# mzhaoshuai/CenterCLIP

Measured on AMD Instinct MI355X. Metric: clips/sec (ViT-B/32, 12f), higher is better.
Workload: dtype fp16 (MFMA operands; fp32 accumulate, residual stream, LN, softmax; cluster + similarity fp32); 1 GPU; cfg2 MSR-VTT-shaped: ViT-B/32 224^2, 12 frames -> 3 segments @block 7, K=49, batch 16, 32 words; global_batch=16, parallelism=single GPU

## Files before the change

### centerclip_amd/csrc/cluster.hip

```cpp
#include "cc_common.h"
#include "cc_kernels.h"

typedef float f32x4 __attribute__((ext_vector_type(4)));

__global__ __launch_bounds__(256) void token_norm_kernel(const float* __restrict__ x, cc_token_layout lay,
                                                         int P, int N, int W, float* __restrict__ sqn,
                                                         float* __restrict__ nrm, float* __restrict__ inv,
                                                         float* __restrict__ xn, int* __restrict__ chunkmax,
                                                         int nchunks) {
    (void)chunkmax; (void)nchunks;
    const int lane = threadIdx.x & 63;
    const int bpp = (N + 3) >> 2;
    const int p = ((int)blockIdx.x >> 3) / bpp * 8 + ((int)blockIdx.x & 7);
    const int j = (((int)blockIdx.x >> 3) % bpp) * 4 + (threadIdx.x >> 6);
    if (p >= P || j >= N) return;
    const int tok = p * N + j;
    const float* src = cc_token_ptr(x, lay, p, j);
    float acc = 0.f;
    for (int w = lane * 4; w < W; w += 256) {
        const float4 v = *reinterpret_cast<const float4*>(src + w);
        acc = fmaf(v.x, v.x, acc);
        acc = fmaf(v.y, v.y, acc);
        acc = fmaf(v.z, v.z, acc);
        acc = fmaf(v.w, v.w, acc);
// ... 448 lines not shown
    return max(max(a, b), max(c, d));
}

__device__ __forceinline__ unsigned cc_wave_umin(unsigned v) {
    v = min(v, (unsigned)__builtin_amdgcn_update_dpp(-1, (int)v, 0xB1, 0xF, 0xF, false));
    v = min(v, (unsigned)__builtin_amdgcn_update_dpp(-1, (int)v, 0x4E, 0xF, 0xF, false));
    v = min(v, (unsigned)__builtin_amdgcn_update_dpp(-1, (int)v, 0x141, 0xF, 0xF, false));
    v = min(v, (unsigned)__builtin_amdgcn_update_dpp(-1, (int)v, 0x140, 0xF, 0xF, false));
    const unsigned a = __builtin_amdgcn_readlane(v, 0), b = __builtin_amdgcn_readlane(v, 16);
    const unsigned c = __builtin_amdgcn_readlane(v, 32), d = __builtin_amdgcn_readlane(v, 48);
    return min(min(a, b), min(c, d));
}

struct GatherDesc {
    const float* x; int64_t in_tok, in_frame;
    int B, T, T_new, n, W, K, mode;
    const long long* medoids; int med_stride;
    const long long* assign;
    const float* cluster_embed;
    const float* cls_mult;
    float* out; int64_t out_tok, out_frame;
    _Float16* h16; float* stats; float* shift;
};
template <bool LEFT>
__device__ void reduce_row_wave(const GatherDesc& g, int row, int lane, const int* med_lds);

struct SelStep {
    const long long* init;
    const int* done;
    int accumulate_iters;
};

#define SEL_WAVES 16
#define SEL_THREADS (64 * SEL_WAVES)
template <bool IN_LDS, int NE>
__global__ __launch_bounds__(SEL_THREADS) void kmedoids_select_kernel(const float* __restrict__ dist_in, float* dist_rw,
                                                              const float* __restrict__ norms,
                                                              const int* __restrict__ chunkmax, int slots_pp, int chunk,
                                                              int apply_shift, int N, int K, int iter_limit,
                                                              int id_sort, long long* __restrict__ medoids_out,
                                                              long long* __restrict__ assign_out,
                                                              int* __restrict__ iters_out, GatherDesc gd, SelStep step) {
    extern __shared__ __attribute__((aligned(16))) unsigned char smem_raw[];
    if (step.done && step.done[(int)blockIdx.x / chunk]) {
        if (step.init != medoids_out)
            for (int k = threadIdx.x; k < K; k += SEL_THREADS) medoids_out[(int64_t)blockIdx.x * K + k] = step.init[(int64_t)blockIdx.x * K + k];
        return;
    }
    const int E = (N + 63) >> 6;
    SelSmem s;
    {
        unsigned char* q = smem_raw;
        s.D = reinterpret_cast<float*>(q);
        if (IN_LDS) q += cc_align_up((size_t)N * N * 4, 8);
        s.best = reinterpret_cast<unsigned long long*>(q); q += cc_align_up((size_t)K * 8, 128);
        s.med = reinterpret_cast<int*>(q); q += cc_align_up((size_t)K * 4, 8);
        s.asg = reinterpret_cast<unsigned short*>(q); q += cc_align_up((size_t)N * 2, 8);
        s.order = reinterpret_cast<unsigned short*>(q); q += cc_align_up((size_t)N * 2, 8);
        s.prev = reinterpret_cast<unsigned short*>(q); q += cc_align_up((size_t)N * 2, 8);
        s.list = reinterpret_cast<unsigned short*>(q); q += cc_align_up((size_t)N * 2, 8);
        s.dirty = reinterpret_cast<unsigned char*>(q); q += cc_align_up((size_t)K, 8);
        s.count = reinterpret_cast<int*>(q); q += 8;
        s.cmask = reinterpret_cast<unsigned long long*>(q); q += (size_t)K * E * 8;
        s.mem = reinterpret_cast<unsigned int*>(q); q += cc_align_up((size_t)N * 4, 8);
        s.cnt = reinterpret_cast<unsigned short*>(q); q += cc_align_up((size_t)K * 2, 8);
        s.off = reinterpret_cast<unsigned short*>(q);
    }
    const int p = blockIdx.x;
    const int tid = threadIdx.x, lane = tid & 63, wave = tid >> 6;
    const int64_t base = (int64_t)p * N * N;
    const float* Dg = dist_in + base;
    SEL_PROF_INIT();
    SEL_STAMP(0);

    float shift_mx = 0.f;
    if (apply_shift) {
        int* red = reinterpret_cast<int*>(smem_raw);
        const int c0 = (p / chunk) * chunk, c1 = min((int)gridDim.x, c0 + chunk);
        int m = (int)0x80000000;
        for (int64_t q = (int64_t)c0 * slots_pp + tid; q < (int64_t)c1 * slots_pp; q += SEL_THREADS) m = max(m, chunkmax[q]);
        m = cc_wave_imax(m);
        if (lane == 0) red[wave] = m;
        __syncthreads();
        int mm = red[0];
#pragma unroll
        for (int w = 1; w < SEL_WAVES; ++w) mm = max(mm, red[w]);
        shift_mx = cc_ordered_int_to_float(mm);
        __syncthreads();
    }
    if (IN_LDS) {
        const float mx = shift_mx;
        float* dst = IN_LDS ? s.D : (dist_rw + base);
        const int total = N * N;
        if (IN_LDS && (total & 3) == 0) {
            const float4* src4 = reinterpret_cast<const float4*>(Dg);
            float4* dst4 = reinterpret_cast<float4*>(dst);
            const int total4 = total >> 2;
            for (int i0 = tid; i0 < total4; i0 += SEL_THREADS * 8) {
                float4 v[8];
#pragma unroll
                for (int u = 0; u < 8; ++u) {
                    const int idx = i0 + u * SEL_THREADS;
                    v[u] = idx < total4 ? src4[idx] : make_float4(0.f, 0.f, 0.f, 0.f);
                }
#pragma unroll
                for (int u = 0; u < 8; ++u) {
                    const int idx = i0 + u * SEL_THREADS;
                    if (idx < total4) {
                        if (apply_shift) {
                            v[u].x = (v[u].x - mx) - 1.0f; v[u].y = (v[u].y - mx) - 1.0f;
                            v[u].z = (v[u].z - mx) - 1.0f; v[u].w = (v[u].w - mx) - 1.0f;
                        }
                        dst4[idx] = v[u];
                    }
                }
            }
        } else {
            for (int i0 = tid; i0 < total; i0 += SEL_THREADS * 8) {
                float v[8];
#pragma unroll
                for (int u = 0; u < 8; ++u) {
                    const int idx = i0 + u * SEL_THREADS;
                    v[u] = idx < total ? Dg[idx] : 0.f;
                }
#pragma unroll
                for (int u = 0; u < 8; ++u) {
                    const int idx = i0 + u * SEL_THREADS;
                    if (idx < total) dst[idx] = apply_shift ? (v[u] - mx) - 1.0f : v[u];
                }
            }
        }
        if (!IN_LDS) Dg = dist_rw + base;
        __threadfence_block();
        __syncthreads();
        if (apply_shift) {
            float* dd = IN_LDS ? s.D : (dist_rw + base);
            for (int i = tid; i < N; i += SEL_THREADS) dd[(int64_t)i * N + i] -= 1.0f;
            __threadfence_block();
        }
        __syncthreads();
    }
    auto dread_global = [&](int i, int j) {
        float d = Dg[(int64_t)i * N + j];
        if (apply_shift) {
            d = (d - shift_mx) - 1.0f;
            if (i == j) d -= 1.0f;
        }
        return d;
    };
#define DREAD(i, j) (IN_LDS ? s.D[(i) * N + (j)] : dread_global((i), (j)))
    SEL_STAMP(1);

    for (int j = tid; j < N; j += SEL_THREADS) s.order[sum_rank(j, N)] = (unsigned short)j;

    if (step.init) {
        for (int k = tid; k < K; k += SEL_THREADS) s.med[k] = (int)step.init[(int64_t)p * K + k];
    } else if (wave == 0) {
        constexpr int TPL = NE;
        float nearest[TPL];
        const float* nr = norms + (int64_t)p * N;
        const int n0 = lane * TPL;
        const float NEG = -__builtin_inff();
#pragma unroll
        for (int e = 0; e < TPL; ++e) nearest[e] = (n0 + e < N) ? nr[n0 + e] : NEG;
        for (int i = 0; i < K; ++i) {
            float loc = nearest[0];
            int slot = 0;
#pragma unroll
            for (int e = 1; e < TPL; ++e)
                if (nearest[e] > loc) { loc = nearest[e]; slot = e; }
            float mx = fmaxf(loc, cc_dpp_f32<0xB1>(loc));
            mx = fmaxf(mx, cc_dpp_f32<0x4E>(mx));
            mx = fmaxf(mx, cc_dpp_f32<0x141>(mx));
            mx = fmaxf(mx, cc_dpp_f32<0x140>(mx));
            {
                const int iv = __float_as_int(mx);
                const float r0 = __int_as_float(__builtin_amdgcn_readlane(iv, 0)), r1 = __int_as_float(__builtin_amdgcn_readlane(iv, 16));
                const float r2 = __int_as_float(__builtin_amdgcn_readlane(iv, 32)), r3 = __int_as_float(__builtin_amdgcn_readlane(iv, 48));
                mx = fmaxf(fmaxf(r0, r1), fmaxf(r2, r3));
            }
            const int src = __ffsll((long long)__ballot(loc == mx)) - 1;
            const int m = src * TPL + __builtin_amdgcn_readlane(slot, src);
            if (lane == 0) s.med[i] = m;
            bool done = false;
            if constexpr (IN_LDS && TPL == 4) {
                if ((N & 3) == 0) {
                    const float4 r = *reinterpret_cast<const float4*>(s.D + m * N + min(n0, N - 4));
                    if (n0 < N) {
                        nearest[0] = (i == 0) ? r.x : fminf(nearest[0], r.x);
                        nearest[1] = (i == 0) ? r.y : fminf(nearest[1], r.y);
                        nearest[2] = (i == 0) ? r.z : fminf(nearest[2], r.z);
                        nearest[3] = (i == 0) ? r.w : fminf(nearest[3], r.w);
                    }
                    done = true;
                }
            }
            if (!done) {
                constexpr int RB = TPL <= 16 ? TPL : 8;
#pragma unroll
                for (int e0 = 0; e0 < TPL; e0 += RB) {
                    float r[RB];
#pragma unroll
                    for (int e = 0; e < RB; ++e) r[e] = (e0 + e < TPL) ? DREAD(m, min(n0 + e0 + e, N - 1)) : 0.f;
#pragma unroll
                    for (int e = 0; e < RB; ++e)
                        if (e0 + e < TPL && n0 + e0 + e < N)
                            nearest[e0 + e] = (i == 0) ? r[e] : fminf(nearest[e0 + e], r[e]);
                }
            }
        }
    }
    __syncthreads();
    SEL_STAMP(2);

    auto assign_step = [&](bool build_masks) {
        if (!IN_LDS && build_masks)
            for (int q = tid; q < K * E; q += SEL_THREADS) s.cmask[q] = 0ull;
        const int part = tid & 3, kq = (K + 3) >> 2;
        const int kb = part * kq, ke = min(K, kb + kq);
        for (int nb = 0; nb < N; nb += SEL_THREADS / 4) {
            const int n = nb + (tid >> 2);
            const int nn = min(n, N - 1);
            float best = __builtin_inff();
            int a = K;
            int k = kb;
            for (; k + 8 <= ke; k += 8) {
                int mk[8];
                float v[8];
#pragma unroll
                for (int u = 0; u < 8; ++u) mk[u] = s.med[k + u];
#pragma unroll
                for (int u = 0; u < 8; ++u) v[u] = DREAD(mk[u], nn);
#pragma unroll
                for (int u = 0; u < 8; ++u)
                    if (v[u] < best || a == K) { best = v[u]; a = k + u; }
            }
            for (; k < ke; ++k) {
                const float v = DREAD(s.med[k], nn);
                if (v < best || a == K) { best = v; a = k; }
            }
#pragma unroll
            for (int o = 1; o <= 2; o <<= 1) {
                const float ob = __shfl_xor(best, o, 64);
                const int oa = __shfl_xor(a, o, 64);
                if (oa < K && (a == K || ob < best || (ob == best && oa < a))) { best = ob; a = oa; }
            }
            if (n < N && part == 0) s.asg[n] = (unsigned short)a;
        }
        if (!IN_LDS && build_masks) {
            __syncthreads();
            for (int t = tid; t < N; t += SEL_THREADS)
                atomicOr(&s.cmask[(size_t)s.asg[s.order[t]] * E + (t >> 6)], 1ull << (t & 63));
        }
    };

    int iters = 0;
    long long ph0 = 0, ph1 = 0, ph2 = 0;
    for (int it = 0; it < iter_limit; ++it) {
        long long tq0 = 0, tq1 = 0, tq2 = 0;
        if (prof) tq0 = (long long)__builtin_readcyclecounter();
        assign_step(true);
        __syncthreads();
        if (prof) tq1 = (long long)__builtin_readcyclecounter();
        for (int k = tid; k < K; k += SEL_THREADS) s.dirty[k] = (it == 0) ? 1 : 0;
        if (tid == 0) *s.count = 0;
        __syncthreads();
        for (int n = tid; n < N; n += SEL_THREADS) {
            const unsigned short a = s.asg[n], pa = s.prev[n];
            if (it > 0 && a != pa) { s.dirty[a] = 1; s.dirty[pa] = 1; }
            s.prev[n] = a;
        }
        __syncthreads();
        if constexpr (!IN_LDS) {
        for (int k = tid; k < K; k += SEL_THREADS) {
            const unsigned long long* cm = s.cmask + (size_t)k * E;
            int n = 0;
            for (int w = 0; w < E; ++w) n += __popcll(cm[w]);
            s.cnt[k] = (unsigned short)n;
            if (s.dirty[k]) s.best[k] = ~0ull;
        }
        __syncthreads();
        if (wave == 0) {
            int carry = 0;
            for (int base = 0; base < K; base += 64) {
                const int v = (base + lane < K) ? (int)s.cnt[base + lane] : 0;
                int incl = v;
#pragma unroll
                for (int o = 1; o < 64; o <<= 1) {
                    const int up = __shfl_up(incl, o, 64);
                    if (lane >= o) incl += up;
                }
                if (base + lane < K) s.off[base + lane] = (unsigned short)(carry + incl - v);
                carry += __shfl(incl, 63, 64);
            }
            if (lane == 0) s.off[K] = (unsigned short)carry;
        }
        __syncthreads();
        const int vec_end = (N < 8) ? 0 : (N & ~7);
        const int rest = (N >> 5) << 5;
        auto tree_code = [&](int j) {
            return ((j & 7) << 7) | (j >= rest ? 31 : ((((j >> 3) & 3) << 5) | (j >> 9)));
        };
        for (int t = tid; t < N; t += SEL_THREADS) {
            const int j = s.order[t];
            const int a = s.asg[j];
            const unsigned long long* cm = s.cmask + (size_t)a * E;
            const int wt = t >> 6;
            unsigned long long below = cm[wt] & ((1ull << (t & 63)) - 1ull);
            int pos = s.off[a] + __popcll(below);
            int tp = below ? 64 * wt + 63 - __clzll((long long)below) : -1;
            for (int w = wt - 1; w >= 0; --w) {
                const unsigned long long m = cm[w];
                pos += __popcll(m);
                if (tp < 0 && m) tp = 64 * w + 63 - __clzll((long long)m);
            }
            unsigned e = (unsigned)j;
            if (j < vec_end) {
                const int jp = tp >= 0 ? (int)s.order[tp] : -1;
                const int x = (jp < 0 || jp >= vec_end) ? 0x3FF : (tree_code(j) ^ tree_code(jp));
                e |= (x ? SEL_F1 : 0u) | ((x >> 5) ? SEL_F2 : 0u) | ((x >> 7) ? SEL_F3 : 0u) | SEL_TREE |
                     (j >= rest ? SEL_LEFT : 0u);
            }
            s.mem[pos] = e;
        }
        __syncthreads();
        if (prof) tq2 = (long long)__builtin_readcyclecounter();
        for (int i = tid; i < N; i += SEL_THREADS) {
            const int cl = s.asg[i];
            if (!s.dirty[cl]) continue;
            const int b0 = s.off[cl], b1 = s.off[cl + 1];
            float c = 0.f, P = 0.f, R = 0.f, F = 0.f;
            for (int q = b0; q < b1; q += 8) {
                int e[8];
                float v[8];
#pragma unroll
                for (int u = 0; u < 8; ++u) e[u] = (q + u < b1) ? (int)s.mem[q + u] : -1;
#pragma unroll
                for (int u = 0; u < 8; ++u) {
                    const float d = DREAD(i, (e[u] < 0 ? 0 : e[u]) & (int)SEL_TOK);
                    v[u] = e[u] < 0 ? 0.f : d;
                }
#pragma unroll
                for (int u = 0; u < 8; ++u) {
                    const int ev = e[u] < 0 ? 0 : e[u];
                    const int m1 = -((ev >> 13) & 1), m2 = -((ev >> 14) & 1), m3 = -((ev >> 15) & 1);
                    const int mt = -((ev >> 16) & 1), ml = -((ev >> 17) & 1);
                    const float t1 = sel_and(c, m1);  P += t1;  c -= t1;
                    const float t2 = sel_and(P, m2);  R += t2;  P -= t2;
                    const float t3 = sel_and(R, m3);  F += t3;  R -= t3;
                    const float vt = sel_and(v[u], mt);
                    const float vl = sel_and(vt, ml);
                    P += vl;
                    c += vt - vl;
                    F += v[u] - vt;
                }
            }
            P += c; R += P; F += R;
            atomicMin(&s.best[cl], ((unsigned long long)cc_float_to_ordered_uint(F) << 32) | (unsigned)i);
        }
        __syncthreads();
        } else {
        for (int k = tid; k < K; k += SEL_THREADS)
            if (s.dirty[k]) s.best[k] = ~0ull;
        for (int n = tid; n < N; n += SEL_THREADS)
            if (s.dirty[s.asg[n]]) s.list[atomicAdd(s.count, 1)] = (unsigned short)n;
        __syncthreads();
        if (prof) tq2 = (long long)__builtin_readcyclecounter();
        {
            const int lq = tid & 7, slot = tid >> 3;
            const int M = *s.count;
            if (N >= 8) {
                const int vec_end = N & ~7, vs = N >> 3, passes = vs >> 2, nleft = vs & 3, ntail = N - vec_end;
                for (int i0 = 0; i0 < M; i0 += SEL_THREADS / 8) {
                    if (i0 + wave * 8 >= M) continue;
                    const int idx = i0 + slot;
                    const int i = s.list[min(idx, M - 1)];
                    const int cl = s.asg[i];
                    float c0[4] = {0.f, 0.f, 0.f, 0.f}, c1[4] = {0.f, 0.f, 0.f, 0.f};
                    const int p0 = min(passes, 16);
#pragma unroll 2
                    for (int it2 = 0; it2 < p0; ++it2) {
                        float d[4];
                        int a4[4];
#pragma unroll
                        for (int k = 0; k < 4; ++k) {
                            const int j = 32 * it2 + 8 * k + lq;
                            d[k] = s.D[i * N + j];
                            a4[k] = s.asg[j];
                        }
#pragma unroll
                        for (int k = 0; k < 4; ++k) c0[k] += (a4[k] == cl) ? d[k] : 0.f;
                    }
#pragma unroll 2
                    for (int it2 = 16; it2 < passes; ++it2) {
                        float d[4];
                        int a4[4];
#pragma unroll
                        for (int k = 0; k < 4; ++k) {
                            const int j = 32 * it2 + 8 * k + lq;
                            d[k] = s.D[i * N + j];
                            a4[k] = s.asg[j];
                        }
#pragma unroll
                        for (int k = 0; k < 4; ++k) c1[k] += (a4[k] == cl) ? d[k] : 0.f;
                    }
                    float P[4];
#pragma unroll
                    for (int k = 0; k < 4; ++k) P[k] = (passes > 16) ? c0[k] + c1[k] : c0[k];
                    for (int v = 0; v < nleft; ++v) {
                        const int j = 32 * passes + 8 * v + lq;
                        const float d = s.D[i * N + j];
                        P[0] += ((int)s.asg[j] == cl) ? d : 0.f;
                    }
                    const float R = ((P[0] + P[1]) + P[2]) + P[3];
                    float F = 0.f;
                    float dt[7];
                    int at[7];
#pragma unroll
                    for (int t = 0; t < 7; ++t) {
                        const int j = min(vec_end + t, N - 1);
                        dt[t] = s.D[i * N + j];
                        at[t] = s.asg[j];
                    }
#pragma unroll
                    for (int t = 0; t < 7; ++t)
                        if (t < ntail) F += (at[t] == cl) ? dt[t] : 0.f;
                    const int base = (tid & 63) & ~7;
                    float r8[8];
#pragma unroll
                    for (int l = 0; l < 8; ++l) r8[l] = __shfl(R, base + l, 64);
#pragma unroll
                    for (int l = 0; l < 8; ++l) F += r8[l];
                    if (lq == 0 && idx < M)
                        atomicMin(&s.best[cl], ((unsigned long long)cc_float_to_ordered_uint(F) << 32) | (unsigned)i);
                }
            } else {
                for (int q = tid; q < M; q += SEL_THREADS) {
                    const int i = s.list[q];
                    const int cl = s.asg[i];
                    float F = 0.f;
                    for (int t = 0; t < N; ++t) {
                        const int j = s.order[t];
                        const float d = DREAD(i, j);
                        F += (s.asg[j] == cl) ? d : 0.f;
                    }
                    atomicMin(&s.best[cl], ((unsigned long long)cc_float_to_ordered_uint(F) << 32) | (unsigned)i);
                }
            }
        }
        __syncthreads();
        }
        int changed = 0;
        for (int k = tid; k < K; k += SEL_THREADS) {
            const unsigned long long b = s.best[k];
            const int bi = (b == ~0ull) ? 0 : (int)(unsigned)(b & 0xFFFFFFFFull);
            changed |= (bi != s.med[k]);
            s.med[k] = bi;
        }
        ++iters;
        const int any_changed = __syncthreads_or(changed);
        if (prof) { ph0 += tq1 - tq0; ph1 += tq2 - tq1; ph2 += (long long)__builtin_readcyclecounter() - tq2; }
        if (!any_changed) break;
    }
    SEL_STAMP(3);

    if (id_sort) {
        int mine = 0, rank = 0;
        if (tid < K) {
            mine = s.med[tid];
            for (int q = 0; q < K; ++q) {
                const int o = s.med[q];
                rank += (o < mine || (o == mine && q < tid)) ? 1 : 0;
            }
        }
        __syncthreads();
        if (tid < K) s.med[rank] = mine;
        __syncthreads();
        if (assign_out) assign_step(false);
        __syncthreads();
    }
    for (int k = tid; k < K; k += SEL_THREADS) medoids_out[(int64_t)p * K + k] = s.med[k];
    if (assign_out)
        for (int n = tid; n < N; n += SEL_THREADS) assign_out[(int64_t)p * N + n] = (iter_limit > 0 || id_sort) ? s.asg[n] : 0;
    if (iters_out && tid == 0) iters_out[p] = step.accumulate_iters ? iters_out[p] + iters : iters;
    if (gd.out) {
        const int b = p % gd.B, sgm = p / gd.B, Lout = 1 + K;
        const int row0 = (b * gd.T_new + sgm) * Lout;
        for (int l = wave; l < Lout; l += SEL_WAVES) reduce_row_wave<false>(gd, row0 + l, lane, s.med);
    }
    SEL_STAMP(4);
    if (prof && tid == 0) {
        prof[(int64_t)blockIdx.x * 16 + 5] = iters;
        prof[(int64_t)blockIdx.x * 16 + 6] = ph0;
        prof[(int64_t)blockIdx.x * 16 + 7] = ph1;
        prof[(int64_t)blockIdx.x * 16 + 8] = ph2;
    }
#undef DREAD
}

struct CascadeSum {
    float4 a0, a1, a2;
    int chunk;
    __device__ __forceinline__ void init() {
        a0 = a1 = a2 = make_float4(0.f, 0.f, 0.f, 0.f);
        chunk = -1;
    }
    static __device__ __forceinline__ void acc(float4& d, const float4& v) { d.x += v.x; d.y += v.y; d.z += v.z; d.w += v.w; }
    __device__ __forceinline__ void close_chunk(int next_chunk) {
        acc(a1, a0);
        a0 = make_float4(0.f, 0.f, 0.f, 0.f);
        if ((chunk >> 4) != (next_chunk >> 4)) { acc(a2, a1); a1 = make_float4(0.f, 0.f, 0.f, 0.f); }
    }
    __device__ __forceinline__ void add(int row, const float4& v) {
        const int c = row >> 4;
        if (chunk >= 0 && c != chunk) close_chunk(c);
        chunk = c;
        acc(a0, v);
    }
    __device__ __forceinline__ float4 total(int rows) {
        if (chunk >= 0 && chunk < (rows >> 4)) {
            const int next = ((chunk >> 4) < (rows >> 8)) ? chunk + 16 : chunk;
            close_chunk(next);
        }
        float4 r = a0;
        acc(r, a1);
        acc(r, a2);
        return r;
    }
};

template <bool LEFT>
struct OuterSum {
    CascadeSum s0;
    CascadeSum s1, s2, s3;
    float4 l0, l1, l2;
    bool ilp;
    int rows4;
    __device__ __forceinline__ void init(bool left_columns, int rows) {
        s0.init();
        ilp = LEFT && left_columns;
        rows4 = (rows >> 2) << 2;
        if (LEFT) {
            s1.init(); s2.init(); s3.init();
            l0 = l1 = l2 = make_float4(0.f, 0.f, 0.f, 0.f);
        }
    }
    __device__ __forceinline__ void add(int row, const float4& v) {
        if (!LEFT || !ilp) { s0.add(row, v); return; }
        if (row >= rows4) {
            const int t = row - rows4;
            if (t == 0) l0 = v; else if (t == 1) l1 = v; else l2 = v;
            return;
        }
        const int a = row & 3, r = row >> 2;
        if (a == 0) s0.add(r, v); else if (a == 1) s1.add(r, v); else if (a == 2) s2.add(r, v); else s3.add(r, v);
    }
    __device__ __forceinline__ float4 total(int rows) {
        if (!LEFT || !ilp) return s0.total(rows);
        const int size = rows >> 2;
        float4 r = s0.total(size);
        CascadeSum::acc(r, l0); CascadeSum::acc(r, l1); CascadeSum::acc(r, l2);
        float4 t = s1.total(size); CascadeSum::acc(r, t);
        t = s2.total(size); CascadeSum::acc(r, t);
        t = s3.total(size); CascadeSum::acc(r, t);
        return r;
    }
};

__global__ __launch_bounds__(256) void cross_dist_kernel(const float* __restrict__ x1, const float* __restrict__ x2, int N1,
                                                         int N2, int W, int metric, float p, float* __restrict__ dist,
                                                         unsigned* __restrict__ gmax) {
    __shared__ float a[16][65], b[16][65];
    const int tid = threadIdx.x, ti = tid >> 4, tj = tid & 15;
    const int bz = blockIdx.z, i0 = blockIdx.y * 16, j0 = blockIdx.x * 16;
    const float* X = x1 + (int64_t)bz * N1 * W;
    const float* Y = x2 + (int64_t)bz * N2 * W;
    const bool gram = metric == CC_METRIC_COSINE || p == 2.0f;
    float dot = 0.f, nx = 0.f, ny = 0.f, lp = 0.f;
    for (int k0 = 0; k0 < W; k0 += 64) {
        for (int e = tid; e < 16 * 64; e += 256) {
            const int r = e >> 6, c = e & 63;
            a[r][c] = (i0 + r < N1 && k0 + c < W) ? X[(int64_t)(i0 + r) * W + k0 + c] : 0.f;
            b[r][c] = (j0 + r < N2 && k0 + c < W) ? Y[(int64_t)(j0 + r) * W + k0 + c] : 0.f;
        }
        __syncthreads();
        const int kn = min(64, W - k0);
        if (gram) {
            for (int c = 0; c < kn; ++c) {
                const float u = a[ti][c], v = b[tj][c];
                dot += u * v; nx += u * u; ny += v * v;
            }
        } else if (p == 1.0f) {
            for (int c = 0; c < kn; ++c) lp += fabsf(a[ti][c] - b[tj][c]);
        } else {
            for (int c = 0; c < kn; ++c) lp += powf(fabsf(a[ti][c] - b[tj][c]), p);
        }
        __syncthreads();
    }
    float d;
    if (metric == CC_METRIC_COSINE) d = 1.0f - dot / ((sqrtf(nx) + 1e-6f) * (sqrtf(ny) + 1e-6f));
    else if (p == 2.0f) d = sqrtf(fmaxf((nx + ny) - 2.f * dot, 0.f));
    else d = (p == 1.0f) ? lp : powf(lp, 1.0f / p);
    const bool in = i0 + ti < N1 && j0 + tj < N2;
    if (in) dist[((int64_t)bz * N1 + i0 + ti) * N2 + j0 + tj] = d;
    if (gmax) {
        float m = in ? d : -__builtin_inff();
        m = cc_wave_max(m);
        if ((tid & 63) == 0) atomicMax(gmax, cc_float_to_ordered_uint(m));
    }
}

__global__ __launch_bounds__(256) void cross_shift_kernel(float* __restrict__ dist, int P, int N1, int N2,
                                                          const unsigned* __restrict__ gmax, int self_nearest) {
    float mx = 0.f;
    if (gmax) {
        const unsigned u = *gmax;
        mx = __uint_as_float((u & 0x80000000u) ? (u & 0x7fffffffu) : ~u);
    }
    const int64_t total = (int64_t)P * N1 * N2;
    for (int64_t idx = (int64_t)blockIdx.x * 256 + threadIdx.x; idx < total; idx += (int64_t)gridDim.x * 256) {
        const int j = (int)(idx % N2);
        const int i = (int)((idx / N2) % N1);
        float v = dist[idx];
        if (gmax) v = (v - mx) - 1.0f;
        if (self_nearest && i == j) v -= 1.0f;
        dist[idx] = v;
    }
}

template <bool LEFT>
__device__ void reduce_row_wave(const GatherDesc& gd, int row, int lane, const int* med_lds) {
    const float* __restrict__ x = gd.x;
    const int64_t in_tok = gd.in_tok, in_frame = gd.in_frame, out_tok = gd.out_tok, out_frame = gd.out_frame;
    const int B = gd.B, T = gd.T, T_new = gd.T_new, n = gd.n, W = gd.W, K = gd.K, mode = gd.mode;
    const long long* __restrict__ medoids = gd.medoids;
    const int med_stride = gd.med_stride;
    const long long* __restrict__ assign = gd.assign;
    const float* __restrict__ cluster_embed = gd.cluster_embed;
    const float* __restrict__ cls_mult = gd.cls_mult;
    float* __restrict__ out = gd.out;
    _Float16* __restrict__ h16 = gd.h16;
    float* __restrict__ stats = gd.stats;
    float* __restrict__ shift = gd.shift;
    const int Lout = (mode == 2) ? 1 + n : 1 + K;
    float st_t = 0.f;
    float* own_row = nullptr;
    auto emit = [&](int w, const float4& v) {
        (void)w;
// ... 88 lines not shown
            a.x = a.x / den; a.y = a.y / den; a.z = a.z / den; a.w = a.w / den;
            if (emb) {
                const float4 e = *reinterpret_cast<const float4*>(emb + w);
                a.x += e.x; a.y += e.y; a.z += e.z; a.w += e.w;
            }
            *reinterpret_cast<float4*>(dst + w) = a;
            emit(w, a);
        }
    }
    finish();
}

template <bool LEFT>
__global__ __launch_bounds__(256) void reduce_tokens_kernel(GatherDesc gd) {
    const int row = blockIdx.x * 4 + (threadIdx.x >> 6);
    const int Lout = (gd.mode == 2) ? 1 + gd.n : 1 + gd.K;
    if (row >= gd.B * gd.T_new * Lout) return;
    reduce_row_wave<LEFT>(gd, row, threadIdx.x & 63, nullptr);
}

static GatherDesc gather_desc(const float* x, int64_t in_tok, int64_t in_frame, int B, int T, int T_new, int n, int W, int K,
                              int mode, const long long* medoids, int med_stride, const long long* assign,
                              const float* cluster_embed, const float* cls_mult, float* out, int64_t out_tok,
                              int64_t out_frame, _Float16* h16, float* stats, float* shift) {
    GatherDesc g{};
    g.x = x; g.in_tok = in_tok; g.in_frame = in_frame;
    g.B = B; g.T = T; g.T_new = T_new; g.n = n; g.W = W; g.K = K; g.mode = mode;
    g.medoids = medoids; g.med_stride = med_stride; g.assign = assign;
    g.cluster_embed = cluster_embed; g.cls_mult = cls_mult;
    g.out = out; g.out_tok = out_tok; g.out_frame = out_frame;
    g.h16 = h16; g.stats = stats; g.shift = shift;
    return g;
}

static void launch_reduce_tokens(hipStream_t st, const float* x, int64_t in_tok, int64_t in_frame, int B, int T, int T_new,
                                 int n, int W, int K, int mode, const long long* medoids, int med_stride,
                                 const long long* assign, const float* cluster_embed, const float* cls_mult, float* out,
                                 int64_t out_tok, int64_t out_frame, _Float16* h16, float* stats, float* shift) {
    const GatherDesc g = gather_desc(x, in_tok, in_frame, B, T, T_new, n, W, K, mode, medoids, med_stride, assign,
                                     cluster_embed, cls_mult, out, out_tok, out_frame, h16, stats, shift);
    const int rows = B * T_new * ((mode == 2) ? 1 + n : 1 + K);
    if (W & 31) hipLaunchKernelGGL(reduce_tokens_kernel<true>, dim3((rows + 3) / 4), dim3(256), 0, st, g);
    else hipLaunchKernelGGL(reduce_tokens_kernel<false>, dim3((rows + 3) / 4), dim3(256), 0, st, g);
}

namespace {

struct ClusterWs {
    int* tilemax;
    int slots_pp;
    int* chunkmax;
    float* sqn;
    float* nrm;
    float* inv;
    float* draw;
    float* xn;
    long long* med;
    long long* asg;
    long long* med2;
    int* done;
    size_t total;
};

struct SpectralWs {
    float* lap;
    float* q;
    int k4;
    void* eig;
    size_t eig_bytes;
    void* km;
    size_t km_bytes;
    size_t total;
};
ClusterWs carve(void* ws, int P, int N, int W, int pre_norm, int K_for_med);
extern "C" size_t cc_spectral_embedding_workspace_bytes(int32_t P, int32_t N);
SpectralWs carve_spectral(void* ws, int P, int N, int K) {
    SpectralWs s{};
    size_t off = 0;
    auto take = [&](size_t bytes) {
        void* ptr = ws ? static_cast<char*>(ws) + off : nullptr;
        off += cc_align_up(bytes, 256);
        return ptr;
    };
    s.k4 = (K + 3) / 4 * 4;
    s.lap = static_cast<float*>(take((size_t)P * N * N * sizeof(float)));
    s.q = static_cast<float*>(take((size_t)P * N * s.k4 * sizeof(float)));
    s.eig_bytes = cc_spectral_embedding_workspace_bytes(P, N);
    s.eig = take(s.eig_bytes);
    s.km_bytes = carve(nullptr, P, N, s.k4, 1, N).total;
    s.km = take(s.km_bytes);
    s.total = off;
    return s;
}

ClusterWs carve(void* ws, int P, int N, int W, int pre_norm, int K_for_med) {
    ClusterWs c{};
    size_t off = 0;
    auto take = [&](size_t bytes) {
        void* ptr = ws ? static_cast<char*>(ws) + off : nullptr;
        off += cc_align_up(bytes, 256);
        return ptr;
    };
    {
        const size_t nt = (size_t)(N + GT - 1) / GT;
        c.slots_pp = (int)(nt * (nt + 1) / 2 * 4);
        c.tilemax = static_cast<int*>(take((size_t)P * c.slots_pp * 4));
        c.chunkmax = static_cast<int*>(take((size_t)P * 4));
    }
    c.sqn = static_cast<float*>(take((size_t)P * N * 4));
    c.nrm = static_cast<float*>(take((size_t)P * N * 4));
    c.inv = static_cast<float*>(take((size_t)P * N * 4));
    c.draw = static_cast<float*>(take((size_t)P * N * N * 4));
    c.med = static_cast<long long*>(take((size_t)P * (size_t)K_for_med * 8));
    c.asg = static_cast<long long*>(take((size_t)P * N * 8));
    c.med2 = static_cast<long long*>(take((size_t)P * (size_t)K_for_med * 8));
    c.done = static_cast<int*>(take((size_t)P * 4));
    c.xn = pre_norm ? static_cast<float*>(take((size_t)P * N * W * 4)) : nullptr;
    c.total = off;
    return c;
}

bool layout_ok(const cc_token_layout* l, int W) {
    if (!l || l->B <= 0 || l->S <= 0 || l->fd <= 0 || l->n <= 0) return false;
    if (W <= 0 || (W & 3)) return false;
    return !((l->stride_b | l->stride_s | l->stride_f | l->stride_i) & 3);
}

cc_token_layout contiguous_layout(int P, int N, int W) {
    cc_token_layout l;
    l.B = P; l.S = 1; l.fd = 1; l.n = N;
    l.stride_b = (int64_t)N * W; l.stride_s = 0; l.stride_f = 0; l.stride_i = W;
    return l;
}

int run_distance(const float* x, cc_token_layout lay, int W, int metric, float p, int chunk, int pre_norm,
                 const ClusterWs& c, hipStream_t st) {
    const int P = lay.B * lay.S, N = lay.fd * lay.n;
    const int nb = ((P + 7) / 8) * 8 * ((N + 3) / 4);
    if (pre_norm) {
        hipLaunchKernelGGL(token_norm_kernel, dim3(nb), dim3(256), 0, st, x, lay, P, N, W, c.sqn, c.nrm, c.inv, c.xn,
                           (int*)nullptr, 0);
        x = c.xn;
        lay = contiguous_layout(P, N, W);
    }
    const bool own_norms = (metric == CC_METRIC_COSINE || p == 2.0f);
    if (!own_norms) {
        hipLaunchKernelGGL(token_norm_kernel, dim3(nb), dim3(256), 0, st, x, lay, P, N, W, c.sqn, c.nrm, c.inv,
                           (float*)nullptr, (int*)nullptr, 0);
        CC_LAUNCH_CHECK();
    }
    const int nt = (N + GT - 1) / GT;
    dim3 grid((unsigned)(((P + 7) / 8) * 8 * (nt * (nt + 1) / 2)));
    const size_t gram_smem = (size_t)2 * 2 * 2 * GT * GK * sizeof(_Float16) + 2 * GT * sizeof(float);
    if (metric == CC_METRIC_COSINE || p == 2.0f) {
        static bool configured = false;
        if (!configured) {
            if (hipFuncSetAttribute(reinterpret_cast<const void*>(gram_dist_kernel<CC_METRIC_COSINE>),
                                    hipFuncAttributeMaxDynamicSharedMemorySize, (int)gram_smem) != hipSuccess ||
                hipFuncSetAttribute(reinterpret_cast<const void*>(gram_dist_kernel<CC_METRIC_EUCLIDEAN>),
                                    hipFuncAttributeMaxDynamicSharedMemorySize, (int)gram_smem) != hipSuccess)
                return CC_ERR_HIP;
            configured = true;
        }
    }
    if (metric == CC_METRIC_COSINE) {
        hipLaunchKernelGGL(gram_dist_kernel<CC_METRIC_COSINE>, grid, dim3(256), gram_smem, st, x, lay, N, W, c.sqn, c.nrm,
                           c.inv, own_norms ? 1 : 0, c.draw, c.tilemax, chunk, nt, P);
    } else if (p == 2.0f) {
        hipLaunchKernelGGL(gram_dist_kernel<CC_METRIC_EUCLIDEAN>, grid, dim3(256), gram_smem, st, x, lay, N, W, c.sqn,
                           c.nrm, c.inv, own_norms ? 1 : 0, c.draw, c.tilemax, chunk, nt, P);
    } else if (p == 1.0f) {
        hipLaunchKernelGGL(lp_dist_kernel<1>, grid, dim3(256), 0, st, x, lay, N, W, p, c.draw, c.tilemax, chunk, nt, P);
    } else if (p > 3.0e38f) {
        hipLaunchKernelGGL(lp_dist_kernel<2>, grid, dim3(256), 0, st, x, lay, N, W, p, c.draw, c.tilemax, chunk, nt, P);
    } else {
        hipLaunchKernelGGL(lp_dist_kernel<0>, grid, dim3(256), 0, st, x, lay, N, W, p, c.draw, c.tilemax, chunk, nt, P);
    }
    CC_LAUNCH_CHECK();
    return CC_OK;
}

int run_distance_sq(const float* x, cc_token_layout lay, int W, const ClusterWs& c, hipStream_t st) {
    const int P = lay.B * lay.S, N = lay.fd * lay.n;
    const int nt = (N + GT - 1) / GT;
    dim3 grid((unsigned)(((P + 7) / 8) * 8 * (nt * (nt + 1) / 2)));
    const size_t gram_smem = (size_t)2 * 2 * 2 * GT * GK * sizeof(_Float16) + 2 * GT * sizeof(float);
    static bool configured = false;
    if (!configured) {
        if (hipFuncSetAttribute(reinterpret_cast<const void*>(gram_dist_kernel<CC_METRIC_SQL2>),
                                hipFuncAttributeMaxDynamicSharedMemorySize, (int)gram_smem) != hipSuccess)
            return CC_ERR_HIP;
        configured = true;
    }
    hipLaunchKernelGGL(gram_dist_kernel<CC_METRIC_SQL2>, grid, dim3(256), gram_smem, st, x, lay, N, W, c.sqn, c.nrm, c.inv,
                       1, c.draw, c.tilemax, P, nt, P);
    CC_LAUNCH_CHECK();
    return CC_OK;
}

int run_select(const float* dist_in, float* dist_rw, const float* norms, const int* chunkmax, int slots_pp, int chunk,
               int apply_shift, int P, int N, int K, int iter_limit, int id_sort, long long* med, long long* assign,
               int* iters, hipStream_t st, const GatherDesc* gather = nullptr, const SelStep* step = nullptr) {
    GatherDesc gd{};
    if (gather) gd = *gather;
    SelStep ss{};
    if (step) ss = *step;
    const size_t lds_limit = 160 * 1024;
    const bool in_lds = sel_smem_bytes(N, K, true) <= lds_limit;
    const size_t smem = sel_smem_bytes(N, K, in_lds);
    if (smem > lds_limit || K > SEL_THREADS) return CC_ERR_UNSUPPORTED;
    const int ne = (N + 63) / 64;
#define SEL_LAUNCH(INLDS, NEV)                                                                                         \
    do {                                                                                                               \
        auto kern = kmedoids_select_kernel<INLDS, NEV>;                                                                \
        if (smem > 64 * 1024 && hipFuncSetAttribute(reinterpret_cast<const void*>(kern),                               \
                                                    hipFuncAttributeMaxDynamicSharedMemorySize, (int)smem) != hipSuccess) \
            return CC_ERR_HIP;                                                                                         \
        hipLaunchKernelGGL(kern, dim3(P), dim3(SEL_THREADS), smem, st, dist_in, dist_rw, norms, chunkmax, slots_pp, chunk, apply_shift, \
                           N, K, iter_limit, id_sort, med, assign, iters, gd, ss);                                    \
    } while (0)
    if (in_lds) {
        if (ne <= 1) SEL_LAUNCH(true, 1);
        else if (ne == 2) SEL_LAUNCH(true, 2);
        else if (ne == 3) SEL_LAUNCH(true, 3);
        else SEL_LAUNCH(true, 4);
    } else {
        if (ne <= 4) SEL_LAUNCH(false, 4);
        else if (ne <= 7) SEL_LAUNCH(false, 7);
        else if (ne <= 10) SEL_LAUNCH(false, 10);
        else if (ne <= 16) SEL_LAUNCH(false, 16);
        else if (ne <= 25) SEL_LAUNCH(false, 25);
        else if (ne <= 40) SEL_LAUNCH(false, 40);
        else if (ne <= 64) SEL_LAUNCH(false, 64);
        else SEL_LAUNCH(false, SEL_MAX_E);
    }
#undef SEL_LAUNCH
    CC_LAUNCH_CHECK();
    return CC_OK;
}

template <typename F>
__device__ float aten_row_sum(int n, F term) {
    if (n < 8) {
        float q[4] = {0.f, 0.f, 0.f, 0.f};
        const int s4 = n >> 2;
        for (int i = 0; i < s4; ++i)
#pragma unroll
            for (int k = 0; k < 4; ++k) q[k] += term(4 * i + k);
        for (int t = 4 * s4; t < n; ++t) q[0] += term(t);
        q[0] += q[1]; q[0] += q[2]; q[0] += q[3];
        return q[0];
    }
    const int vs = n >> 3, passes = vs >> 2;
    float a0[32], a1[32];
#pragma unroll
    for (int u = 0; u < 32; ++u) { a0[u] = 0.f; a1[u] = 0.f; }
    int i = 0;
    while (i + 16 <= passes) {
        for (int r = 0; r < 16; ++r, ++i)
#pragma unroll
            for (int u = 0; u < 32; ++u) a0[u] += term(32 * i + u);
#pragma unroll
        for (int u = 0; u < 32; ++u) { a1[u] += a0[u]; a0[u] = 0.f; }
    }
    for (; i < passes; ++i)
#pragma unroll
        for (int u = 0; u < 32; ++u) a0[u] += term(32 * i + u);
#pragma unroll
    for (int u = 0; u < 32; ++u) a0[u] += a1[u];
    for (int v = 4 * passes; v < vs; ++v)
#pragma unroll
        for (int l = 0; l < 8; ++l) a0[l] += term(8 * v + l);
    float out = 0.f;
    for (int t = 8 * vs; t < n; ++t) out += term(t);
#pragma unroll
    for (int l = 0; l < 8; ++l) out += ((a0[l] + a0[8 + l]) + a0[16 + l]) + a0[24 + l];
    return out;
}

__global__ __launch_bounds__(256) void center_shift_kernel(const float* __restrict__ x, cc_token_layout lay, int W, int P, int K,
                                                           int chunk, const long long* __restrict__ med_new,
                                                           const long long* __restrict__ med_prev, float threshold,
                                                           int* __restrict__ done, float* __restrict__ rows_ws) {
    const int c = blockIdx.x, p0 = c * chunk, bc = min(chunk, P - p0);
    if (done[c]) return;
    float* rows = rows_ws + (int64_t)p0 * K;
    for (int r = threadIdx.x; r < bc * K; r += 256) {
        const int b = r / K, k = r - b * K, p = p0 + b;
        const float* xa = cc_token_ptr(x, lay, p, (int)med_new[(int64_t)p * K + k]);
        const float* xb = cc_token_ptr(x, lay, p, (int)med_prev[(int64_t)p * K + k]);
        const float ss = aten_row_sum(W, [&](int j) { const float d = xa[j] - xb[j]; return d * d; });
        rows[r] = sqrtf(ss);
    }
    __threadfence_block();
    __syncthreads();
    __shared__ float per_problem[1024];
    for (int b = threadIdx.x; b < bc; b += 256)
        per_problem[b] = aten_row_sum(K, [&](int k) { return rows[(int64_t)b * K + k]; });
    __syncthreads();
    if (threadIdx.x == 0) {
        const float total = aten_row_sum(bc, [&](int b) { return per_problem[b]; });
        const float shift = total / (float)bc;
        if (shift < threshold) done[c] = 1;
    }
}

bool p_supported(int metric, float p) { return metric == CC_METRIC_COSINE || (p > 0.0f); }

}

extern "C" {

#ifdef CC_DEV_KNOBS
int cc_debug_set_gram_profile(long long* buf) {
    return hipMemcpyToSymbol(HIP_SYMBOL(g_gram_prof), &buf, sizeof(buf)) == hipSuccess ? CC_OK : CC_ERR_HIP;
}
int cc_debug_set_select_profile(long long* buf) {
    return hipMemcpyToSymbol(HIP_SYMBOL(g_sel_prof), &buf, sizeof(buf)) == hipSuccess ? CC_OK : CC_ERR_HIP;
}
#endif

size_t cc_spectral_workspace_bytes(int32_t P, int32_t N, int32_t K) {
    if (P <= 0 || N <= 0 || K <= 0) return 0;
    return carve_spectral(nullptr, P, N, K).total;
}

size_t cc_cluster_workspace_bytes(int32_t P, int32_t N, int32_t W, int32_t pre_norm) {
    if (P <= 0 || N <= 0 || W <= 0) return 0;
    return carve(nullptr, P, N, W, pre_norm, N).total;
}

int cc_token_norms_f32(const float* x, const cc_token_layout* lay, int32_t W, float* norms, void* ws,
                       size_t ws_bytes, void* stream) {
    if (!x || !norms || !layout_ok(lay, W)) return CC_ERR_INVALID;
    const int P = lay->B * lay->S, N = lay->fd * lay->n;
    ClusterWs c = carve(ws, P, N, W, 0, N);
    if (!ws || ws_bytes < c.total) return CC_ERR_WORKSPACE;
    hipLaunchKernelGGL(token_norm_kernel, dim3(((P + 7) / 8) * 8 * ((N + 3) / 4)), dim3(256), 0, static_cast<hipStream_t>(stream), x, *lay,
                       P, N, W, c.sqn, norms, c.inv, (float*)nullptr, (int*)nullptr, 0);
    CC_LAUNCH_CHECK();
    return CC_OK;
}

int cc_pairwise_distance_f32(const float* x, const cc_token_layout* lay, int32_t W, int32_t metric, float p,
                             int32_t all_negative, int32_t self_nearest, int32_t chunk, float* dist,
                             float* norms_out, void* ws, size_t ws_bytes, void* stream) {
// ... 769 lines not shown
```

Before: 8678 clips/s.

## Fuse dirty tracking into k-medoids assign step and exit early on no moves

Dirty and prev tracking now happen inside the assignment pass, which removes a separate pass over N tokens and two block barriers per iteration. The loop exits straight after the assign step when no token changed cluster. Candidate list building uses a wave ballot with one atomic per wave instead of one atomic per token, and the argmax in the init loop becomes a tree max plus a slot search. It also drops the static once-only guard around hipFuncSetAttribute, so that host call now runs on every launch, and adds one extra profiling counter.

```diff
diff --git a/centerclip_amd/csrc/cluster.hip b/centerclip_amd/csrc/cluster.hip
--- a/centerclip_amd/csrc/cluster.hip
+++ b/centerclip_amd/csrc/cluster.hip
@@ -624,6 +624,8 @@
     SEL_STAMP(1);
 
     for (int j = tid; j < N; j += SEL_THREADS) s.order[sum_rank(j, N)] = (unsigned short)j;
+    for (int k = tid; k < K; k += SEL_THREADS) s.dirty[k] = 1;
+    if (tid == 0) *s.count = 0;
 
     if (step.init) {
         for (int k = tid; k < K; k += SEL_THREADS) s.med[k] = (int)step.init[(int64_t)p * K + k];
@@ -637,10 +639,19 @@
         for (int e = 0; e < TPL; ++e) nearest[e] = (n0 + e < N) ? nr[n0 + e] : NEG;
         for (int i = 0; i < K; ++i) {
             float loc = nearest[0];
-            int slot = 0;
-#pragma unroll
-            for (int e = 1; e < TPL; ++e)
-                if (nearest[e] > loc) { loc = nearest[e]; slot = e; }
+            if constexpr (TPL <= 8) {
+                float part[TPL];
+#pragma unroll
+                for (int e = 0; e < TPL; ++e) part[e] = nearest[e];
+#pragma unroll
+                for (int w = 1; w < TPL; w <<= 1)
+#pragma unroll
+                    for (int e = 0; e + w < TPL; e += 2 * w) part[e] = fmaxf(part[e], part[e + w]);
+                loc = part[0];
+            } else {
+#pragma unroll
+                for (int e = 1; e < TPL; ++e) loc = fmaxf(loc, nearest[e]);
+            }
             float mx = fmaxf(loc, cc_dpp_f32<0xB1>(loc));
             mx = fmaxf(mx, cc_dpp_f32<0x4E>(mx));
             mx = fmaxf(mx, cc_dpp_f32<0x141>(mx));
@@ -651,6 +662,9 @@
                 const float r2 = __int_as_float(__builtin_amdgcn_readlane(iv, 32)), r3 = __int_as_float(__builtin_amdgcn_readlane(iv, 48));
                 mx = fmaxf(fmaxf(r0, r1), fmaxf(r2, r3));
             }
+            int slot = TPL - 1;
+#pragma unroll
+            for (int e = TPL - 2; e >= 0; --e) slot = (nearest[e] == mx) ? e : slot;
             const int src = __ffsll((long long)__ballot(loc == mx)) - 1;
             const int m = src * TPL + __builtin_amdgcn_readlane(slot, src);
             if (lane == 0) s.med[i] = m;
@@ -685,14 +699,16 @@
     __syncthreads();
     SEL_STAMP(2);
 
-    auto assign_step = [&](bool build_masks) {
+    auto assign_step = [&](bool build_masks, bool track, bool compare_prev) {
         if (!IN_LDS && build_masks)
             for (int q = tid; q < K * E; q += SEL_THREADS) s.cmask[q] = 0ull;
         const int part = tid & 3, kq = (K + 3) >> 2;
         const int kb = part * kq, ke = min(K, kb + kq);
+        int moved = 0;
         for (int nb = 0; nb < N; nb += SEL_THREADS / 4) {
             const int n = nb + (tid >> 2);
             const int nn = min(n, N - 1);
+            const int pa = compare_prev ? (int)s.prev[nn] : -1;
             float best = __builtin_inff();
             int a = K;
             int k = kb;
@@ -717,32 +733,35 @@
                 const int oa = __shfl_xor(a, o, 64);
                 if (oa < K && (a == K || ob < best || (ob == best && oa < a))) { best = ob; a = oa; }
             }
-            if (n < N && part == 0) s.asg[n] = (unsigned short)a;
+            if (n < N && part == 0) {
+                s.asg[n] = (unsigned short)a;
+                if (track) {
+                    s.prev[n] = (unsigned short)a;
+                    if (compare_prev && a != pa) { s.dirty[a] = 1; s.dirty[pa] = 1; moved = 1; }
+                }
+            }
         }
         if (!IN_LDS && build_masks) {
             __syncthreads();
             for (int t = tid; t < N; t += SEL_THREADS)
                 atomicOr(&s.cmask[(size_t)s.asg[s.order[t]] * E + (t >> 6)], 1ull << (t & 63));
         }
+        return moved;
     };
 
     int iters = 0;
-    long long ph0 = 0, ph1 = 0, ph2 = 0;
+    long long ph0 = 0, ph1 = 0, ph2 = 0, ph3 = 0;
     for (int it = 0; it < iter_limit; ++it) {
-        long long tq0 = 0, tq1 = 0, tq2 = 0;
+        long long tq0 = 0, tq1 = 0, tq2 = 0, tq3 = 0;
         if (prof) tq0 = (long long)__builtin_readcyclecounter();
-        assign_step(true);
-        __syncthreads();
+        const int moved = assign_step(true, true, it > 0);
+        const int any_moved = __syncthreads_or(moved);
         if (prof) tq1 = (long long)__builtin_readcyclecounter();
-        for (int k = tid; k < K; k += SEL_THREADS) s.dirty[k] = (it == 0) ? 1 : 0;
-        if (tid == 0) *s.count = 0;
-        __syncthreads();
-        for (int n = tid; n < N; n += SEL_THREADS) {
-            const unsigned short a = s.asg[n], pa = s.prev[n];
-            if (it > 0 && a != pa) { s.dirty[a] = 1; s.dirty[pa] = 1; }
-            s.prev[n] = a;
-        }
-        __syncthreads();
+        if (it > 0 && !any_moved) {
+            ++iters;
+            if (prof) ph0 += tq1 - tq0;
+            break;
+        }
         if constexpr (!IN_LDS) {
         for (int k = tid; k < K; k += SEL_THREADS) {
             const unsigned long long* cm = s.cmask + (size_t)k * E;
@@ -834,8 +853,17 @@
         } else {
         for (int k = tid; k < K; k += SEL_THREADS)
             if (s.dirty[k]) s.best[k] = ~0ull;
-        for (int n = tid; n < N; n += SEL_THREADS)
-            if (s.dirty[s.asg[n]]) s.list[atomicAdd(s.count, 1)] = (unsigned short)n;
+        for (int nb = wave * 64; nb < N; nb += SEL_THREADS) {
+            const int n = nb + lane;
+            const bool cand = n < N && s.dirty[s.asg[min(n, N - 1)]];
+            const unsigned long long bal = __ballot(cand);
+            if (bal) {
+                int at = 0;
+                if (lane == 0) at = atomicAdd(s.count, __popcll(bal));
+                at = __builtin_amdgcn_readfirstlane(at);
+                if (cand) s.list[at + __popcll(bal & ((1ull << lane) - 1ull))] = (unsigned short)n;
+            }
+        }
         __syncthreads();
         if (prof) tq2 = (long long)__builtin_readcyclecounter();
         {
@@ -922,16 +950,22 @@
         }
         __syncthreads();
         }
+        if (prof) tq3 = (long long)__builtin_readcyclecounter();
         int changed = 0;
         for (int k = tid; k < K; k += SEL_THREADS) {
             const unsigned long long b = s.best[k];
             const int bi = (b == ~0ull) ? 0 : (int)(unsigned)(b & 0xFFFFFFFFull);
             changed |= (bi != s.med[k]);
             s.med[k] = bi;
-        }
+            s.dirty[k] = 0;
+        }
+        if (tid == 0) *s.count = 0;
         ++iters;
         const int any_changed = __syncthreads_or(changed);
-        if (prof) { ph0 += tq1 - tq0; ph1 += tq2 - tq1; ph2 += (long long)__builtin_readcyclecounter() - tq2; }
+        if (prof) {
+            const long long tq4 = (long long)__builtin_readcyclecounter();
+            ph0 += tq1 - tq0; ph1 += tq2 - tq1; ph2 += tq4 - tq2; ph3 += tq4 - tq3;
+        }
         if (!any_changed) break;
     }
     SEL_STAMP(3);
@@ -948,7 +982,7 @@
         __syncthreads();
         if (tid < K) s.med[rank] = mine;
         __syncthreads();
-        if (assign_out) assign_step(false);
+        if (assign_out) assign_step(false, false, false);
         __syncthreads();
     }
     for (int k = tid; k < K; k += SEL_THREADS) medoids_out[(int64_t)p * K + k] = s.med[k];
@@ -966,6 +1000,7 @@
         prof[(int64_t)blockIdx.x * 16 + 6] = ph0;
         prof[(int64_t)blockIdx.x * 16 + 7] = ph1;
         prof[(int64_t)blockIdx.x * 16 + 8] = ph2;
+        prof[(int64_t)blockIdx.x * 16 + 9] = ph3;
     }
 #undef DREAD
 }
@@ -1360,16 +1395,14 @@
     const int nt = (N + GT - 1) / GT;
     dim3 grid((unsigned)(((P + 7) / 8) * 8 * (nt * (nt + 1) / 2)));
     const size_t gram_smem = (size_t)2 * 2 * 2 * GT * GK * sizeof(_Float16) + 2 * GT * sizeof(float);
-    if (metric == CC_METRIC_COSINE || p == 2.0f) {
-        static bool configured = false;
-        if (!configured) {
-            if (hipFuncSetAttribute(reinterpret_cast<const void*>(gram_dist_kernel<CC_METRIC_COSINE>),
-                                    hipFuncAttributeMaxDynamicSharedMemorySize, (int)gram_smem) != hipSuccess ||
-                hipFuncSetAttribute(reinterpret_cast<const void*>(gram_dist_kernel<CC_METRIC_EUCLIDEAN>),
-                                    hipFuncAttributeMaxDynamicSharedMemorySize, (int)gram_smem) != hipSuccess)
-                return CC_ERR_HIP;
-            configured = true;
-        }
+    if (metric == CC_METRIC_COSINE) {
+        if (hipFuncSetAttribute(reinterpret_cast<const void*>(gram_dist_kernel<CC_METRIC_COSINE>),
+                                hipFuncAttributeMaxDynamicSharedMemorySize, (int)gram_smem) != hipSuccess)
+            return CC_ERR_HIP;
+    } else if (p == 2.0f) {
+        if (hipFuncSetAttribute(reinterpret_cast<const void*>(gram_dist_kernel<CC_METRIC_EUCLIDEAN>),
+                                hipFuncAttributeMaxDynamicSharedMemorySize, (int)gram_smem) != hipSuccess)
+            return CC_ERR_HIP;
     }
     if (metric == CC_METRIC_COSINE) {
         hipLaunchKernelGGL(gram_dist_kernel<CC_METRIC_COSINE>, grid, dim3(256), gram_smem, st, x, lay, N, W, c.sqn, c.nrm,
@@ -1393,13 +1426,9 @@
     const int nt = (N + GT - 1) / GT;
     dim3 grid((unsigned)(((P + 7) / 8) * 8 * (nt * (nt + 1) / 2)));
     const size_t gram_smem = (size_t)2 * 2 * 2 * GT * GK * sizeof(_Float16) + 2 * GT * sizeof(float);
-    static bool configured = false;
-    if (!configured) {
-        if (hipFuncSetAttribute(reinterpret_cast<const void*>(gram_dist_kernel<CC_METRIC_SQL2>),
-                                hipFuncAttributeMaxDynamicSharedMemorySize, (int)gram_smem) != hipSuccess)
-            return CC_ERR_HIP;
-        configured = true;
-    }
+    if (hipFuncSetAttribute(reinterpret_cast<const void*>(gram_dist_kernel<CC_METRIC_SQL2>),
+                            hipFuncAttributeMaxDynamicSharedMemorySize, (int)gram_smem) != hipSuccess)
+        return CC_ERR_HIP;
     hipLaunchKernelGGL(gram_dist_kernel<CC_METRIC_SQL2>, grid, dim3(256), gram_smem, st, x, lay, N, W, c.sqn, c.nrm, c.inv,
                        1, c.draw, c.tilemax, P, nt, P);
     CC_LAUNCH_CHECK();
```

Measured after the change: 8678 clips/s (median of 3 runs). Within noise of the previous version (-0.0%).
